# PrioteasaAndrei/music-style-transfer-ldm

Measured on AMD Instinct MI355X. Metric: UNet denoising steps/sec on 1×128×512 mel-latents, 1/2/4/8 MI355X, higher is better.
Workload: dtype fp32; 1 GPU; config 2: 50-step DDIM reverse sample (49 UNet+update iterations per step), batch 8/GPU, 1x128x512 mel -> [8,32,16,64] latents, eta=0.0, hipGraph replay of 1 concurrent sub-batch chains; global_batch=8, parallelism=dp1 (batch shards)

## Files before the change

include/ldm_capi.h:

```cpp
#ifndef LDM_CAPI_H
#define LDM_CAPI_H

#include <stddef.h>
#include <stdint.h>

#ifdef __cplusplus
extern "C" {
#endif

#define LDM_CAPI_VERSION 1

const char* ldm_last_error(void);
int ldm_capi_version(void);
int ldm_device_count(int* count);

typedef struct ldm_conv_desc {
    int32_t B, Cin, Hin, Win;
    int32_t Cout, Hout, Wout;
    int32_t kh, kw, stride, pad, out_pad;
    int32_t transposed;
    int32_t layout;
} ldm_conv_desc;

enum {
// ... 19 lines not shown
    float bn_eps;
    int32_t act;
    const float* bcast_add;
    const float* skip_add;
    float* act_out;
    int32_t dtype;
} ldm_epilogue;

typedef struct ldm_conv_plan {
    int32_t kind;
    int32_t tm, tn, wk;
    int32_t ks;
    int32_t balance;
    int64_t packed_floats;
    int64_t ws_floats;
} ldm_conv_plan;

int ldm_conv_make_plan(const ldm_conv_desc* d, ldm_conv_plan* plan);
int ldm_conv_tiled_plan(const ldm_conv_desc* d, int32_t dtype, ldm_conv_plan* plan);
int ldm_conv_sconv_plan(const ldm_conv_desc* d, int32_t dtype, ldm_conv_plan* plan);
int ldm_conv_make_plan_forced(const ldm_conv_desc* d, int kind, int tm, int tn, int wk, int ks,
                              ldm_conv_plan* plan);
int ldm_conv_pack_weight(const ldm_conv_desc* d, const ldm_conv_plan* plan, const float* w,
                         float* packed, void* stream);
int32_t ldm_conv_storage16(const ldm_conv_desc* d, const ldm_conv_plan* plan);
int ldm_conv_forward(const ldm_conv_desc* d, const ldm_conv_plan* plan, const float* x, const float* w,
                     const ldm_epilogue* ep, float* y, void* stream);
int ldm_conv_forward_ws(const ldm_conv_desc* d, const ldm_conv_plan* plan, const float* x, const float* w,
                        const ldm_epilogue* ep, float* y, float* workspace, void* stream);

int64_t ldm_reduce_workspace_floats(int32_t B, int32_t C, int32_t HW);
int ldm_batchnorm_train(float* x, int32_t B, int32_t C, int32_t HW, const float* weight, const float* bias,
                        float* running_mean, float* running_var, float momentum, float eps, int32_t act,
                        float* save_mean, float* save_invstd, float* workspace, void* stream);
int ldm_batchnorm_train_out(const float* x, float* y, int32_t B, int32_t C, int32_t HW, const float* weight,
                            const float* bias, float* running_mean, float* running_var, float momentum, float eps,
                            int32_t act, float* save_mean, float* save_invstd, float* workspace, void* stream);
int ldm_batchnorm_stats(const float* x, int32_t B, int32_t C, int32_t HW, double* stats, float* workspace,
                        void* stream);
int ldm_batchnorm_stats_code(const float* x, int32_t code, int32_t B, int32_t C, int32_t HW, double* stats,
                             float* workspace, void* stream);
int ldm_batchnorm_apply(float* x, int32_t B, int32_t C, int32_t HW, const double* stats, double count,
                        const float* weight, const float* bias, float* running_mean, float* running_var,
                        float momentum, float eps, int32_t act, float* save_mean, float* save_invstd, void* stream);
int ldm_batchnorm_apply_out(const float* x, float* y, int32_t B, int32_t C, int32_t HW, const double* stats,
                            double count, const float* weight, const float* bias, float* running_mean,
                            float* running_var, float momentum, float eps, int32_t act, float* save_mean,
                            float* save_invstd, void* stream);

int ldm_batchnorm_eval(const float* x, float* y, int32_t B, int32_t C, int32_t HW, const float* weight,
                       const float* bias, const float* running_mean, const float* running_var, float eps, int32_t act,
                       void* stream);

int ldm_activation(const float* x, float* y, int64_t n, int32_t act, void* stream);

int ldm_sinusoid_embed(const void* t, int32_t t_is_float, int32_t B, int32_t dim, const float* freqs, float* out,
                       void* stream);

int ldm_time_mlp_forward(const void* t, int32_t t_is_float, int32_t B, int32_t dim, const float* freqs,
                         const float* w1, const float* b1, const float* w2, const float* b2, float* out,
                         void* stream);

int ldm_attention_fold_keys(const float* kv, const float* wq, const float* bq, int32_t B, int32_t E, int32_t heads,
                            int32_t S, float scale, float* kf, float* bf, void* stream);
int ldm_attention_folded(const float* z, const float* kv, const float* kf, const float* bf, float* out, int32_t B,
                         int32_t E, int32_t heads, int32_t L, int32_t S, void* stream);
int ldm_attention_folded_keys(const float* z, const float* kv, const float* kf, const float* bf,
                              const float* key_bias, float* out, int32_t B, int32_t E, int32_t heads, int32_t L,
                              int32_t S, void* stream);
int ldm_attention_fold_keys_bias(const float* kv, const float* wq, const float* bq, int32_t B, int32_t E,
                                 int32_t heads, int32_t S, float scale, const float* key_bias, float* kf, float* bf,
                                 void* stream);
int ldm_attention_folded_probs(const float* z, const float* kf, const float* bf, float* p, int32_t B, int32_t E,
                               int32_t heads, int32_t L, int32_t S, void* stream);
int32_t ldm_bneck_fold_supported(int32_t B, int32_t H, int32_t W);
int ldm_bneck_fold_values(const float* w_fold, const float* kv, float* u, int32_t B, void* stream);
int ldm_bneck_pv(const float* u, const float* p, const float* pos_bias, float* y, int32_t B, int32_t dtype,
                 void* stream);
int ldm_ca1_probs(const float* z4, const float* kf, const float* bf, float* p, int32_t B, void* stream);
int32_t ldm_ca1_probs_form(void);
int ldm_set_cin1_packed(int on);
int ldm_set_cin1_s1(int on);
int ldm_set_flash_split(int on);
int ldm_fold_conv_proj(const ldm_conv_desc* d, const float* w_conv, const float* b_conv, const float* w_proj,
                       const float* b_proj, int32_t Cmid, float* w_out, float* pos_bias_out, void* stream);
int ldm_attention_core(const float* q, const float* kv, float* out, int32_t B, int32_t E, int32_t heads,
                       int32_t L, int32_t S, float scale, void* stream);
int ldm_attention_flash_supported(int32_t E, int32_t heads);
int ldm_attention_forward_lse(const float* q, const float* kv, float* out, float* lse, int32_t B, int32_t E,
                              int32_t heads, int32_t L, int32_t S, float scale, void* stream);

int ldm_q_sample(const float* x0, const float* eps, const float* coef_table, int32_t T, const int64_t* t, float* zt,
                 int32_t B, int64_t per_sample, void* stream);
int ldm_predict_start(const float* zt, const float* eps, const float* coef_table, int32_t T, const int64_t* t,
                      float* x0, int32_t B, int64_t per_sample, void* stream);
int ldm_sched_backward(int32_t kind, const float* grad, const float* coef_table, int32_t T, const int64_t* t,
                       float* grad_a, float* grad_b, int32_t B, int64_t per_sample, void* stream);
int ldm_ddim_step(float* x, const float* eps, const float* coef, float eta, float* x0_log, float* eps_log,
                  int64_t n, void* stream);
int ldm_msolver_step(float* x, const float* eps, const float* coef, const float* x0_prev, float* x0_log,
                     float* eps_log, int64_t n, void* stream);

int ldm_loss_forward(int32_t kind, const float* a, const float* b, int64_t n, void* workspace, float* out,
                     void* stream);
int ldm_loss_backward(int32_t kind, const float* a, const float* b, int64_t n, const float* grad_out, float* grad_a,
                      float* grad_b, void* stream);

typedef struct ldm_unet_weights {
    const float* conv_w[9];
    const float* conv_b[9];
    ldm_conv_plan conv_plan[9];
    const float* ca_wq[2];
    const float* ca_bq[2];
    ldm_conv_plan ca_plan_q[2];
    const float* ca_wkv[2];
    const float* ca_bkv[2];
    ldm_conv_plan ca_plan_kv[2];
    const float* ca_wo[2];
    const float* ca_bo[2];
    ldm_conv_plan ca_plan_o[2];
    const float* t_freqs;
    const float* t_w1;
    const float* t_b1;
    const float* t_w2;
    const float* t_b2;
    const float* ca_wq_raw[2];
    const float* fold_w[2];
    const float* fold_pb[2];
    int32_t use_fold;
    const float* step_w[9];
    const float* step_pb[2];
    int32_t use_step;
    int32_t step_dtype;
    const float* step_bneck_w;
} ldm_unet_weights;

typedef struct ldm_unet_shape {
    int32_t B, C, H, W;
    int32_t nf;
} ldm_unet_shape;

int64_t ldm_unet_workspace_floats(const ldm_unet_shape* s, const ldm_unet_weights* w);
int ldm_unet_make_plans(const ldm_unet_shape* s, ldm_unet_weights* w);
int ldm_unet_layer_desc(const ldm_unet_shape* s, int32_t layer, ldm_conv_desc* d);
int ldm_unet_forward(const ldm_unet_shape* s, const ldm_unet_weights* w, const float* z, const void* t,
                     int32_t t_is_float, const float* s5, const float* s6, float* out, float* workspace,
                     void* stream);

int64_t ldm_ddim_workspace_floats(const ldm_unet_shape* s, const ldm_unet_weights* w, int32_t nsteps);
int ldm_ddim_sample(const ldm_unet_shape* s, const ldm_unet_weights* w, float* x, const float* s5,
                    const float* s6, const int64_t* t_table, const float* coef_table, int32_t nsteps, float eta,
                    float* x0_logs, float* eps_logs, int64_t log_step_stride, float* workspace, void* stream);
int ldm_msolver_sample(const ldm_unet_shape* s, const ldm_unet_weights* w, float* x, const float* s5,
                       const float* s6, const int64_t* t_table, const float* coef_table, int32_t nsteps,
                       float* x0_logs, float* eps_logs, int64_t log_step_stride, float* workspace, void* stream);
int64_t ldm_ddim_workspace_floats_mix(const ldm_unet_shape* s, const ldm_unet_weights* w, int32_t nsteps, int32_t S5,
                                      int32_t S6);
int ldm_ddim_sample_mix(const ldm_unet_shape* s, const ldm_unet_weights* w, float* x, const float* s5,
                        const float* s6, int32_t S5, int32_t S6, const float* key_bias5, const float* key_bias6,
                        const int64_t* t_table, const float* coef_table, int32_t nsteps, float eta, float* x0_logs,
                        float* eps_logs, int64_t log_step_stride, float* workspace, void* stream);
int ldm_msolver_sample_mix(const ldm_unet_shape* s, const ldm_unet_weights* w, float* x, const float* s5,
                           const float* s6, int32_t S5, int32_t S6, const float* key_bias5, const float* key_bias6,
                           const int64_t* t_table, const float* coef_table, int32_t nsteps, float* x0_logs,
                           float* eps_logs, int64_t log_step_stride, float* workspace, void* stream);
int64_t ldm_ddim_workspace_floats_guided(const ldm_unet_shape* s, const ldm_unet_weights* w, int32_t nsteps, int32_t S5,
// ... 177 lines not shown
```

music-style-transfer-ldm_amd/csrc/misc.hip:

```cpp
#include <algorithm>

#include "common.h"

#pragma clang fp contract(off)

namespace ldm {

__global__ __launch_bounds__(256) void time_mlp_kernel(const void* t, int t_is_float, int dim, const float* __restrict__ freqs,
                                                       const float* __restrict__ w1, const float* __restrict__ b1,
                                                       const float* __restrict__ w2, const float* __restrict__ b2,
                                                       float* __restrict__ out) {
    extern __shared__ __attribute__((aligned(16))) float sm[];
    float* emb = sm;
    float* hid = sm + dim;
    const int b = blockIdx.x, i = threadIdx.x;
    const float tv = t_is_float ? ((const float*)t)[b] : (float)((const int64_t*)t)[b];
    const int half = dim / 2;
    if (i < dim) {
        const float arg = tv * freqs[i < half ? i : i - half];
        emb[i] = i < half ? sinf(arg) : cosf(arg);
    }
    __syncthreads();
    if (i < dim) {
        const float* wr = w1 + (size_t)i * dim;
// ... 232 lines not shown

#pragma unroll
        for (int r = 0; r < MF::NACC; ++r) Ps[(lt * TILE + MF::row(r, lg)) * LDP + st * TILE + col] = acc[r];
    }
    __syncthreads();
    {
        constexpr int RPW = SP >= 64 ? 1 : 64 / SP;
        constexpr int SEG = SP >= 64 ? 64 : SP;
        const int sub = lane / SEG, s0 = lane % SEG;
        for (int r0 = wave * RPW; r0 < LT; r0 += NW * RPW) {
            const int r = r0 + sub;
            float* row = Ps + r * LDP;
            float x[SP / SEG];
            float mx = -INFINITY;
#pragma unroll
            for (int u = 0; u < SP / SEG; ++u) {
                const int s = s0 + u * SEG;
                if constexpr (EQ > 0) {
                    float v = row[s];
#pragma unroll
                    for (int w = 1; w < NW; ++w) v = v + row[s + w * LT * LDP];
                    x[u] = v + (s < S ? bf[(size_t)(b * heads + h) * S + s] : 0.f);
                } else {
                    x[u] = row[s];
                }
                if (s < S) mx = fmaxf(mx, x[u]);
            }
#pragma unroll
            for (int o = SEG / 2; o > 0; o >>= 1) mx = fmaxf(mx, __shfl_xor(mx, o));
            float sum = 0.f;
#pragma unroll
            for (int u = 0; u < SP / SEG; ++u) {
                const int s = s0 + u * SEG;
                x[u] = s < S ? expf(x[u] - mx) : 0.f;
                sum += x[u];
            }
#pragma unroll
            for (int o = SEG / 2; o > 0; o >>= 1) sum += __shfl_xor(sum, o);
#pragma unroll
            for (int u = 0; u < SP / SEG; ++u) row[s0 + u * SEG] = l0 + r < L ? x[u] / sum : 0.f;
        }
    }
    __syncthreads();
    if constexpr (PONLY) {
        float* pb = out + ((size_t)(b * heads + h) * L + l0) * S;
        for (int e = threadIdx.x; e < LT * SP; e += 64 * NW) {
            const int r = e / SP, s = e % SP;
            if (l0 + r < L && s < S) pb[(size_t)r * S + s] = Ps[r * LDP + s];
        }
        return;
    }
    constexpr int NTC = D / TILE;
    float* ob = TOK ? out + (size_t)b * L * E + (size_t)h * D : out + ((size_t)b * E + (size_t)h * D) * L;
    for (int tile = wave; tile < NTC * NTL; tile += NW) {
        const int ct = tile / NTL, lt = tile % NTL;
        typename MF::acc_t acc;
#pragma unroll
        for (int r = 0; r < MF::NACC; ++r) acc[r] = 0.f;
        const float* va = Vs + (ct * TILE + col) * LDP + lg;
        const float* pb = Ps + (lt * TILE + col) * LDP + lg;
#pragma unroll
        for (int k0 = 0; k0 < SP; k0 += KBP * NLG) {
            float av[KBP], bv[KBP];
#pragma unroll
            for (int j = 0; j < KBP; ++j) {
                av[j] = va[k0 + NLG * j];
                bv[j] = pb[k0 + NLG * j];
            }
#pragma unroll
            for (int j = 0; j < KBP; ++j) acc = MF::mma(av[j], bv[j], acc);
        }
        const int l = l0 + lt * TILE + col;
        if (l < L) {
            if constexpr (TOK && KIND == 2) {
                *reinterpret_cast<float4*>(ob + (size_t)l * E + ct * TILE + 4 * lg) = make_float4(acc[0], acc[1], acc[2], acc[3]);
            } else {
#pragma unroll
                for (int r = 0; r < MF::NACC; ++r) ob[(ct * TILE + MF::row(r, lg)) * qcs + l * qls] = acc[r];
            }
        }
    }
}

__global__ __launch_bounds__(256) void attention_fold_keys_kernel(const float* __restrict__ kv, const float* __restrict__ wq,
                                                                  const float* __restrict__ bq, int B, int E, int heads,
                                                                  int S, float scale, float* __restrict__ kf,
                                                                  float* __restrict__ bf, int64_t first) {
    const int d = E / heads;
    const int64_t nk = (int64_t)B * heads * E * S;
    const int64_t idx = first + (int64_t)blockIdx.x * blockDim.x + threadIdx.x;
    if (idx < nk) {
        const int e = (int)(idx % E);
        int64_t r = idx / E;
        const int s = (int)(r % S);
        r /= S;
        const int h = (int)(r % heads), b = (int)(r / heads);
        const float* kr = kv + ((int64_t)b * 2 * E + (int64_t)h * d) * S + s;
        const float* wr = wq + (int64_t)h * d * E + e;
        double acc = 0.0;
        int c = 0;
        for (; c + 16 <= d; c += 16) {
            float wv[16], kvv[16];
#pragma unroll
            for (int u = 0; u < 16; ++u) {
                wv[u] = wr[(int64_t)(c + u) * E];
                kvv[u] = kr[(int64_t)(c + u) * S];
            }
#pragma unroll
            for (int u = 0; u < 16; ++u) acc += (double)wv[u] * (double)kvv[u];
        }
        for (; c < d; ++c) acc += (double)wr[(int64_t)c * E] * (double)kr[(int64_t)c * S];
        kf[idx] = (float)(acc * (double)scale);
    } else if (idx < nk + (int64_t)B * heads * S) {
        const int64_t j = idx - nk;
        const int s = (int)(j % S);
        const int bh = (int)(j / S);
        const int h = bh % heads, b = bh / heads;
        const float* kr = kv + ((int64_t)b * 2 * E + (int64_t)h * d) * S + s;
        double acc = 0.0;
        for (int c = 0; c < d; ++c) acc += (double)bq[h * d + c] * (double)kr[(int64_t)c * S];
        bf[j] = (float)(acc * (double)scale);
    }
}

__global__ __launch_bounds__(256) void attention_fold_keys4_kernel(const float* __restrict__ kv, const float* __restrict__ wq,
                                                                   const float* __restrict__ bq, int B, int E, int heads,
                                                                   int S, float scale, float* __restrict__ kf,
                                                                   float* __restrict__ bf) {
    const int d = E / heads;
    const int SG = S / 4;
    const int64_t n = (int64_t)B * heads * SG * (E + 1);
    const int64_t idx = (int64_t)blockIdx.x * blockDim.x + threadIdx.x;
    if (idx >= n) return;
    const int e = (int)(idx % (E + 1));
    int64_t r = idx / (E + 1);
    const int sg = (int)(r % SG);
    r /= SG;
    const int h = (int)(r % heads), b = (int)(r / heads);
    const float* kr = kv + ((int64_t)b * 2 * E + (int64_t)h * d) * S + sg * 4;
    const bool isb = e == E;
    const float* wr = isb ? bq + h * d : wq + (int64_t)h * d * E + e;
    const int64_t ws = isb ? 1 : E;
    double acc[4] = {0., 0., 0., 0.};
    int c = 0;
    for (; c + 16 <= d; c += 16) {
        float wv[16];
        float4 kq[16];
#pragma unroll
        for (int u = 0; u < 16; ++u) {
            wv[u] = wr[(int64_t)(c + u) * ws];
            kq[u] = *reinterpret_cast<const float4*>(kr + (int64_t)(c + u) * S);
        }
#pragma unroll
        for (int u = 0; u < 16; ++u) {
            const double w = (double)wv[u];
            acc[0] += w * (double)kq[u].x;
            acc[1] += w * (double)kq[u].y;
            acc[2] += w * (double)kq[u].z;
            acc[3] += w * (double)kq[u].w;
        }
    }
    for (; c < d; ++c) {
        const double w = (double)wr[(int64_t)c * ws];
        const float4 k = *reinterpret_cast<const float4*>(kr + (int64_t)c * S);
        acc[0] += w * (double)k.x;
        acc[1] += w * (double)k.y;
// ... 158 lines not shown
                                                       const float* __restrict__ freqs, float* __restrict__ out) {
    const int i = blockIdx.x * blockDim.x + threadIdx.x;
    if (i >= B * dim) return;
    const int b = i / dim, k = i - b * dim, half = dim / 2;
    const float tv = t_is_float ? ((const float*)t)[b] : (float)((const int64_t*)t)[b];
    const float arg = tv * freqs[k < half ? k : k - half];
    out[i] = k < half ? sinf(arg) : cosf(arg);
}

constexpr int kLossBlocks = 512;

__device__ __forceinline__ float loss_term(int kind, float a, float b) {
    if (kind == 0) {
        const float d = a - b;
        return d * d;
    }
    const float a2 = a * a;
    return 0.5f * ((a2 - 1.0f) - logf(a2 + 1e-8f));
}

__global__ __launch_bounds__(256) void loss_partial_kernel(int kind, const float* __restrict__ a,
                                                           const float* __restrict__ b, int64_t n,
                                                           double* __restrict__ partial) {
    __shared__ double red[16];
    double s = 0.0;
    for (int64_t i = (int64_t)blockIdx.x * blockDim.x + threadIdx.x; i < n; i += (int64_t)gridDim.x * blockDim.x)
        s += (double)loss_term(kind, a[i], b ? b[i] : 0.f);
    for (int o = 32; o > 0; o >>= 1) s += __shfl_xor(s, o);
    const int lane = threadIdx.x & 63, wave = threadIdx.x >> 6;
    if (lane == 0) red[wave] = s;
    __syncthreads();
    if (threadIdx.x == 0) {
        double t = 0.0;
        for (int w = 0; w < (int)(blockDim.x >> 6); ++w) t += red[w];
        partial[blockIdx.x] = t;
    }
}

__global__ __launch_bounds__(64) void loss_final_kernel(const double* __restrict__ partial, int np, int64_t n,
                                                        float* __restrict__ out) {
    double s = 0.0;
    for (int i = threadIdx.x; i < np; i += 64) s += partial[i];
    for (int o = 32; o > 0; o >>= 1) s += __shfl_xor(s, o);
    if (threadIdx.x == 0) out[0] = (float)(s / (double)n);
}

__global__ __launch_bounds__(256) void loss_backward_kernel(int kind, const float* __restrict__ a,
                                                            const float* __restrict__ b, int64_t n,
                                                            const float* __restrict__ g, float* __restrict__ ga,
                                                            float* __restrict__ gb) {
    const int64_t i = (int64_t)blockIdx.x * blockDim.x + threadIdx.x;
    if (i >= n) return;
    const float scale = g[0] / (float)n;
    if (kind == 0) {
        const float d = 2.0f * (a[i] - (b ? b[i] : 0.f)) * scale;
        if (ga) ga[i] = d;
        if (gb) gb[i] = -d;
    } else {
        const float av = a[i];
        const float a2 = av * av;
        if (ga) ga[i] = (av - av / (a2 + 1e-8f)) * scale;
    }
}

static unsigned blocks_for(int64_t n, int t) { return (unsigned)((n + t - 1) / t); }

}

using namespace ldm;

extern "C" int ldm_time_mlp_forward(const void* t, int32_t t_is_float, int32_t B, int32_t dim, const float* freqs,
                                    const float* w1, const float* b1, const float* w2, const float* b2, float* out,
                                    void* stream) {
    LDM_REQUIRE(t && freqs && w1 && b1 && w2 && b2 && out, "time_mlp: null argument");
    LDM_REQUIRE(B > 0 && dim > 1 && dim % 2 == 0 && dim <= 256, "time_mlp: unsupported dim");
    const int threads = (dim + 63) / 64 * 64;
    hipLaunchKernelGGL(time_mlp_kernel, dim3(B), dim3(threads), 2 * dim * sizeof(float), (hipStream_t)stream, t,
                       t_is_float, dim, freqs, w1, b1, w2, b2, out);
    LDM_CHECK_LAUNCH("time_mlp_kernel");
    return 0;
}

namespace ldm {
int attention_folded(const float* z, const float* kv, const float* kf, const float* bf, float* out, int32_t B,
                     int32_t E, int32_t heads, int32_t L, int32_t S, hipStream_t st) {
    LDM_REQUIRE(z && kv && kf && bf && out, "attention (folded): null argument");
    LDM_REQUIRE(B > 0 && heads == 4 && L > 0 && S > 0, "attention (folded): bad shape");
    const int d = E / heads;
#define LDM_ATTF(LP, SP, D, LT, EQV, NWV)                                                                \
    if (d == D && E == EQV && L <= LP && S <= SP) {                                                      \
        const size_t lds = ((size_t)NWV * LT * (SP + 1) + (size_t)D * (SP + 1)) * sizeof(float);       \
        if (lds > 64 * 1024) {                                                                           \
            static bool opted = false;                                                                   \
            if (!opted) {                                                                                \
                LDM_HIP_TRY(hipFuncSetAttribute(                                                         \
                    (const void*)attention_mfma_kernel<2, LP, SP, D, LT, true, EQV, NWV>,                  \
                    hipFuncAttributeMaxDynamicSharedMemorySize, 160 * 1024));                            \
                opted = true;                                                                            \
            }                                                                                            \
        }                                                                                                \
        hipLaunchKernelGGL((attention_mfma_kernel<2, LP, SP, D, LT, true, EQV, NWV>), dim3(B * heads * (LP / LT)), \
                           dim3(64 * NWV), lds, st, z, kv, out, E, heads, L, S, 1.0f, kf, bf);           \
        LDM_CHECK_LAUNCH("attention_mfma_kernel (folded)");                                              \
        return 0;                                                                                        \
    }
    LDM_ATTF(16, 16, 128, 16, 512, 8)
    LDM_ATTF(64, 64, 64, 16, 256, 16)
    LDM_ATTF(32, 32, 64, 16, 256, 8)
    LDM_ATTF(32, 32, 128, 16, 512, 8)
    LDM_ATTF(16, 16, 64, 16, 256, 4)
#undef LDM_ATTF
    return fail(3, "attention (folded): no instance for this shape");
}

int attention_folded_probs(const float* z, const float* kf, const float* bf, float* p, int32_t B, int32_t E,
                           int32_t heads, int32_t L, int32_t S, hipStream_t st) {
    LDM_REQUIRE(z && kf && bf && p, "attention probs (folded): null argument");
    LDM_REQUIRE(B > 0 && heads == 4 && E == 512 && L > 0 && L <= 16 && S > 0 && S <= 16,
                "attention probs (folded): instances for CA1's 2 x 8 plane only (E 512, L, S <= 16)");
    static const int nw = [] {
        const char* e = std::getenv("LDM_CA1P_WAVES");
        return e && std::atoi(e) == 16 ? 16 : 8;
    }();
    if (nw == 16) {
        auto kfn = attention_mfma_kernel<2, 16, 16, 128, 16, true, 512, 16, true>;
        const size_t lds = ((size_t)16 * 16 * 17 + (size_t)128 * 17) * sizeof(float);
        hipLaunchKernelGGL(kfn, dim3(B * heads), dim3(64 * 16), lds, st, z, kf, p, E, heads, L, S, 1.0f, kf, bf);
    } else {
        auto kfn = attention_mfma_kernel<2, 16, 16, 128, 16, true, 512, 8, true>;
        const size_t lds = ((size_t)8 * 16 * 17 + (size_t)128 * 17) * sizeof(float);
        hipLaunchKernelGGL(kfn, dim3(B * heads), dim3(64 * 8), lds, st, z, kf, p, E, heads, L, S, 1.0f, kf, bf);
    }
    LDM_CHECK_LAUNCH("attention_mfma_kernel (folded, probabilities)");
    return 0;
}

int attention_fold_keys(const float* kv, const float* wq, const float* bq, int32_t B, int32_t E, int32_t heads,
                        int32_t S, float scale, float* kf, float* bf, hipStream_t st) {
    LDM_REQUIRE(kv && wq && bq && kf && bf && B > 0 && heads > 0 && E % heads == 0 && S > 0, "fold keys: bad argument");
    const int64_t nk = (int64_t)B * heads * E * S, nb = (int64_t)B * heads * S;
    static const bool k4_on = [] {
        const char* e = std::getenv("LDM_FOLD_KEYS4");
        return e ? std::atoi(e) != 0 : true;
    }();
    const bool k4 = k4_on && S % 4 == 0 && ((uintptr_t)kv & 15) == 0;
    if (k4) {
        const int64_t n4 = (int64_t)B * heads * (S / 4) * (E + 1);
        hipLaunchKernelGGL(attention_fold_keys4_kernel, dim3((unsigned)((n4 + 255) / 256)), dim3(256), 0, st, kv, wq, bq,
                           B, E, heads, S, scale, kf, bf);
        LDM_CHECK_LAUNCH("attention_fold_keys4_kernel");
        return 0;
    }
    const int64_t first = 0, n = nk + nb - first;
    hipLaunchKernelGGL(attention_fold_keys_kernel, dim3((unsigned)((n + 255) / 256)), dim3(256), 0, st, kv, wq, bq, B,
                       E, heads, S, scale, kf, bf, first);
    LDM_CHECK_LAUNCH("attention_fold_keys_kernel");
    return 0;
}

int attention_core_ex(const float* q, const float* kv, float* out, int32_t B, int32_t E, int32_t heads, int32_t L,
                      int32_t S, float scale, bool tok, hipStream_t st) {
    LDM_REQUIRE(q && kv && out, "attention: null argument");
    LDM_REQUIRE(B > 0 && heads > 0 && E % heads == 0 && L > 0 && S > 0, "attention: bad shape");
    const int d = E / heads;
    {
        const dim3 blk(256);
#define LDM_ATT(KIND, LP, SP, D, LT)                                                                      \
    if (d == D && L <= LP && S <= SP) {                                                                   \
        const size_t lds = ((size_t)LT * (SP + 1) + (size_t)D * (SP + 1)) * sizeof(float);              \
        if (tok)                                                                                          \
            hipLaunchKernelGGL((attention_mfma_kernel<KIND, LP, SP, D, LT, true>), dim3(B * heads * (LP / LT)), blk, \
// ... 69 lines not shown
    return 0;
}

extern "C" int ldm_msolver_step(float* x, const float* eps, const float* coef, const float* x0_prev, float* x0_log,
                                float* eps_log, int64_t n, void* stream) {
    LDM_REQUIRE(x && eps && coef && x0_log && n > 0, "msolver_step: bad argument");
    LDM_REQUIRE(x0_prev != x0_log, "msolver_step: x0_prev must not be the x0 output");
    hipLaunchKernelGGL(msolver_step_kernel, dim3(blocks_for(n, 256)), dim3(256), 0, (hipStream_t)stream, x, eps, coef,
                       x0_prev, x0_log, eps_log, n);
    LDM_CHECK_LAUNCH("msolver_step_kernel");
    return 0;
}

extern "C" int ldm_guide_eps(const float* e_t, const float* e_b, const float* scale, int64_t per_sample, int32_t B,
                             float* out, void* stream) {
    LDM_REQUIRE(e_t && e_b && scale && out && per_sample > 0 && B > 0, "guide_eps: bad argument");
    const int64_t n = per_sample * B;
    hipLaunchKernelGGL(guide_eps_kernel, dim3(blocks_for(n, 256)), dim3(256), 0, (hipStream_t)stream, e_t, e_b, scale,
                       per_sample, n, out);
    LDM_CHECK_LAUNCH("guide_eps_kernel");
    return 0;
}

extern "C" int ldm_activation(const float* x, float* y, int64_t n, int32_t act, void* stream) {
    LDM_REQUIRE(x && y && n >= 0, "activation: bad argument");
    if (n == 0) return 0;
    hipLaunchKernelGGL(activation_kernel, dim3(blocks_for(n, 256)), dim3(256), 0, (hipStream_t)stream, x, y, n, act);
    LDM_CHECK_LAUNCH("activation_kernel");
    return 0;
}

extern "C" int ldm_batchnorm_eval(const float* x, float* y, int32_t B, int32_t C, int32_t HW, const float* weight,
                                  const float* bias, const float* running_mean, const float* running_var, float eps,
                                  int32_t act, void* stream) {
    LDM_REQUIRE(x && y && running_mean && running_var && B > 0 && C > 0 && HW > 0, "batchnorm_eval: bad argument");
    const int64_t n = (int64_t)B * C * HW;
    hipLaunchKernelGGL(batchnorm_eval_kernel, dim3(blocks_for(n, 256)), dim3(256), 0, (hipStream_t)stream, x, y, C, HW,
                       n, weight, bias, running_mean, running_var, eps, act);
    LDM_CHECK_LAUNCH("batchnorm_eval_kernel");
    return 0;
}

extern "C" int ldm_sinusoid_embed(const void* t, int32_t t_is_float, int32_t B, int32_t dim, const float* freqs,
                                  float* out, void* stream) {
    LDM_REQUIRE(t && freqs && out && B > 0 && dim > 1 && dim % 2 == 0, "sinusoid: bad argument");
    hipLaunchKernelGGL(sinusoid_kernel, dim3(blocks_for((int64_t)B * dim, 256)), dim3(256), 0, (hipStream_t)stream, t,
                       t_is_float, B, dim, freqs, out);
    LDM_CHECK_LAUNCH("sinusoid_kernel");
    return 0;
}

extern "C" int ldm_loss_forward(int32_t kind, const float* a, const float* b, int64_t n, void* workspace, float* out,
                                void* stream) {
    LDM_REQUIRE(a && workspace && out && n > 0 && (kind == 0 || kind == 1), "loss_forward: bad argument");
    LDM_REQUIRE(kind != 0 || b, "loss_forward: mse needs two inputs");
    const int np = (int)std::min<int64_t>(kLossBlocks, (n + 255) / 256);
    hipLaunchKernelGGL(loss_partial_kernel, dim3(np), dim3(256), 0, (hipStream_t)stream, kind, a, b, n,
                       (double*)workspace);
    LDM_CHECK_LAUNCH("loss_partial_kernel");
    hipLaunchKernelGGL(loss_final_kernel, dim3(1), dim3(64), 0, (hipStream_t)stream, (const double*)workspace, np, n, out);
    LDM_CHECK_LAUNCH("loss_final_kernel");
    return 0;
}

extern "C" int ldm_loss_backward(int32_t kind, const float* a, const float* b, int64_t n, const float* grad_out,
                                 float* grad_a, float* grad_b, void* stream) {
    LDM_REQUIRE(a && grad_out && n > 0 && (kind == 0 || kind == 1), "loss_backward: bad argument");
    hipLaunchKernelGGL(loss_backward_kernel, dim3(blocks_for(n, 256)), dim3(256), 0, (hipStream_t)stream, kind, a, b, n,
                       grad_out, grad_a, grad_b);
    LDM_CHECK_LAUNCH("loss_backward_kernel");
    return 0;
}

extern "C" int ldm_attention_fold_keys(const float* kv, const float* wq, const float* bq, int32_t B, int32_t E,
                                       int32_t heads, int32_t S, float scale, float* kf, float* bf, void* stream) {
    return ldm::attention_fold_keys(kv, wq, bq, B, E, heads, S, scale, kf, bf, (hipStream_t)stream);
}

extern "C" int ldm_attention_folded(const float* z, const float* kv, const float* kf, const float* bf, float* out,
                                    int32_t B, int32_t E, int32_t heads, int32_t L, int32_t S, void* stream) {
    return ldm::attention_folded(z, kv, kf, bf, out, B, E, heads, L, S, (hipStream_t)stream);
}

extern "C" int ldm_attention_folded_probs(const float* z, const float* kf, const float* bf, float* p, int32_t B,
                                          int32_t E, int32_t heads, int32_t L, int32_t S, void* stream) {
    return ldm::attention_folded_probs(z, kf, bf, p, B, E, heads, L, S, (hipStream_t)stream);
}

extern "C" int ldm_fold_conv_proj(const ldm_conv_desc* d, const float* w_conv, const float* b_conv, const float* w_proj,
                                  const float* b_proj, int32_t Cmid, float* w_out, float* pos_bias_out, void* stream) {
    LDM_REQUIRE(d && w_conv && w_proj && b_proj && w_out && pos_bias_out, "fold conv/proj: null argument");
    LDM_REQUIRE(!d->transposed && d->kh * d->kw > 0 && Cmid > 0, "fold conv/proj: a plain conv after the projection");
    const int64_t n = (int64_t)d->Cout * d->Cin * d->kh * d->kw + (int64_t)d->Cout * d->Hout * d->Wout;
    hipLaunchKernelGGL(ldm::fold_conv_proj_kernel, dim3((unsigned)((n + 255) / 256)), dim3(256), 0, (hipStream_t)stream,
                       w_conv, b_conv, w_proj, b_proj, d->Cout, Cmid, d->Cin, d->kh, d->kw, d->stride, d->pad, d->Hin,
                       d->Win, d->Hout, d->Wout, w_out, pos_bias_out);
    LDM_CHECK_LAUNCH("fold_conv_proj_kernel");
    return 0;
}
```

music-style-transfer-ldm_amd/ldm_amd/_lib.py:

```python
import ctypes
import os

import torch

PKG_ROOT = os.path.dirname(os.path.dirname(os.path.abspath(__file__)))
LIB_PATH = os.environ.get("LDM_AMD_LIB", os.path.join(PKG_ROOT, "lib", "libldm_amd.so"))

c_int32 = ctypes.c_int32
c_int64 = ctypes.c_int64
c_float = ctypes.c_float
c_vp = ctypes.c_void_p
c_fp = ctypes.c_void_p


class ConvDesc(ctypes.Structure):
    _fields_ = [(n, c_int32) for n in
                ("B", "Cin", "Hin", "Win", "Cout", "Hout", "Wout", "kh", "kw", "stride", "pad", "out_pad", "transposed",
                 "layout")]

    def key(self):
        return tuple(getattr(self, f[0]) for f in self._fields_)


class Epilogue(ctypes.Structure):
# ... 62 lines not shown
    "ldm_step_layer_forms": (c_int32, [c_vp]),
    "ldm_step_dec1_ddim": (c_int32, [c_int32, c_int32, c_int32, c_fp, c_fp, c_fp, c_fp, c_float, c_fp, c_fp, c_fp,
                                     c_int32, c_vp]),
    "ldm_step_dec1_msolver": (c_int32, [c_int32, c_int32, c_int32, c_fp, c_fp, c_fp, c_fp, c_fp, c_fp, c_fp, c_fp,
                                        c_int32, c_vp]),
    "ldm_step_conv_ws": (c_int32, [c_int32, c_int32, c_int32, c_int32, c_fp, c_fp, c_fp, c_fp, c_fp, c_fp, c_int32,
                                   c_fp, c_vp]),
    "ldm_mel_quantize": (c_int32, [c_fp, c_fp, c_int64, ctypes.c_float, c_vp]),
    "ldm_mel_dequantize": (c_int32, [c_fp, c_fp, c_int64, ctypes.c_float, c_vp]),
    "ldm_u8_to_unit": (c_int32, [c_fp, c_fp, c_int64, c_vp]),
    "ldm_stft_table_floats": (c_int64, [c_int32]),
    "ldm_stft_fill_tables": (c_int32, [c_int32, c_vp]),
    "ldm_stft": (c_int32, [c_fp, c_int32, c_int64, c_int32, c_int32, c_fp, c_fp, c_fp, c_int32, c_vp]),
    "ldm_istft": (c_int32, [c_fp, c_fp, c_fp, c_int32, c_int32, c_int64, c_int32, c_int32, c_fp, c_vp]),
    "ldm_griffinlim_workspace": (c_int64, [c_int32, c_int32, c_int32]),
    "ldm_griffinlim": (c_int32, [c_fp, c_fp, c_fp, c_int32, c_int32, c_int64, c_int32, c_int32, c_int32, c_float,
                                 c_fp, c_fp, c_vp]),
    "ldm_mel_project": (c_int32, [c_fp, c_fp, c_vp, c_fp, c_int32, c_int32, c_int32, c_int32, c_vp]),
    "ldm_power_to_db": (c_int32, [c_fp, c_fp, c_int32, c_int64, c_float, c_float, c_fp, c_vp]),
    "ldm_db_to_power": (c_int32, [c_fp, c_fp, c_int64, c_vp]),
    "ldm_mel_invert": (c_int32, [c_fp, c_fp, c_fp, c_fp, c_vp, c_float, c_int32, c_int32, c_fp, c_fp, c_int32,
                                 c_int32, c_int32, c_int32, c_vp]),
    "ldm_resample_out_len": (c_int64, [c_int64, c_int32, c_int32]),
    "ldm_resample_f32": (c_int32, [c_fp, c_int32, c_int64, c_fp, c_int32, c_int32, c_int32, c_fp, c_vp]),
    "ldm_resample_pcm16": (c_int32, [c_vp, c_int64, c_int32, c_fp, c_int32, c_int32, c_int32, c_fp, c_vp]),
    "ldm_trim_workspace_floats": (c_int64, [c_int32, c_int64, c_int32]),
    "ldm_trim_bounds": (c_int32, [c_fp, c_int32, c_int64, c_int32, c_int32, c_float, c_fp, c_vp, c_vp]),
    "ldm_mel_window_count": (c_int64, [c_int64, c_int32, c_int32]),
    "ldm_mel_windows": (c_int32, [c_fp, c_int32, c_int64, c_int32, c_int32, c_float, c_float, c_float, c_fp, c_fp,
                                  c_vp]),
    "ldm_mel_stitch": (c_int32, [c_fp, c_fp, c_int32, c_int32, c_int32, c_int32, c_int64, c_float, c_fp, c_fp, c_vp]),
    "ldm_batchnorm_train": (c_int32, [c_fp, c_int32, c_int32, c_int32, c_fp, c_fp, c_fp, c_fp, c_float, c_float,
                                      c_int32, c_fp, c_fp, c_fp, c_vp]),
    "ldm_batchnorm_train_out": (c_int32, [c_fp, c_fp, c_int32, c_int32, c_int32, c_fp, c_fp, c_fp, c_fp, c_float,
                                          c_float, c_int32, c_fp, c_fp, c_fp, c_vp]),
    "ldm_batchnorm_apply_out": (c_int32, [c_fp, c_fp, c_int32, c_int32, c_int32, c_vp, ctypes.c_double, c_fp, c_fp,
                                          c_fp, c_fp, c_float, c_float, c_int32, c_fp, c_fp, c_vp]),
    "ldm_maxpool2x2": (c_int32, [c_fp, c_fp, c_int32, c_int32, c_int32, c_int32, c_vp]),
    "ldm_std_mse_workspace_floats": (c_int64, [c_int32, c_int64]),
    "ldm_std_mse_moments": (c_int32, [c_fp, c_fp, c_int32, c_int64, c_vp, c_fp, c_vp]),
    "ldm_std_mse_accumulate": (c_int32, [c_vp, c_int32, c_int64, ctypes.c_double, ctypes.c_double, c_vp, c_fp, c_vp]),
    "ldm_batchnorm_stats": (c_int32, [c_fp, c_int32, c_int32, c_int32, c_vp, c_fp, c_vp]),
    "ldm_batchnorm_apply": (c_int32, [c_fp, c_int32, c_int32, c_int32, c_vp, ctypes.c_double, c_fp, c_fp, c_fp, c_fp,
                                      c_float, c_float, c_int32, c_fp, c_fp, c_vp]),
    "ldm_batchnorm_eval": (c_int32, [c_fp, c_fp, c_int32, c_int32, c_int32, c_fp, c_fp, c_fp, c_fp, c_float, c_int32,
                                     c_vp]),
    "ldm_activation": (c_int32, [c_fp, c_fp, c_int64, c_int32, c_vp]),
    "ldm_sinusoid_embed": (c_int32, [c_vp, c_int32, c_int32, c_int32, c_fp, c_fp, c_vp]),
    "ldm_time_mlp_forward": (c_int32, [c_vp, c_int32, c_int32, c_int32, c_fp, c_fp, c_fp, c_fp, c_fp, c_fp, c_vp]),
    "ldm_attention_core": (c_int32, [c_fp, c_fp, c_fp, c_int32, c_int32, c_int32, c_int32, c_int32, c_float, c_vp]),
    "ldm_attention_flash_supported": (c_int32, [c_int32, c_int32]),
    "ldm_attention_forward_lse": (c_int32, [c_fp, c_fp, c_fp, c_fp, c_int32, c_int32, c_int32, c_int32, c_int32,
                                            c_float, c_vp]),
    "ldm_attention_backward_flash": (c_int32, [c_fp, c_fp, c_fp, c_fp, c_fp, c_fp, c_fp, c_fp, c_int32, c_int32,
                                               c_int32, c_int32, c_int32, c_float, c_vp]),
    "ldm_pack_job_bytes": (c_int64, []),
    "ldm_pack_many_prepare": (c_int32, [ctypes.POINTER(ConvDesc), ctypes.POINTER(ConvPlan), ctypes.POINTER(c_vp),
                                        ctypes.POINTER(c_vp), c_int32, c_vp, ctypes.POINTER(c_int64)]),
    "ldm_pack_many": (c_int32, [c_vp, c_int32, c_int64, c_vp]),
    "ldm_im2col": (c_int32, [c_fp, c_int32, c_int32, c_int32, c_int32, c_int32, c_int32, c_int32, c_int32, c_int32,
                             c_fp, c_fp, c_int32, c_int32, c_fp, c_vp]),
    "ldm_col2im": (c_int32, [c_fp, c_int32, c_int32, c_int32, c_int32, c_int32, c_int32, c_int32, c_int32, c_int32,
                             c_fp, c_int32, c_int32, c_fp, c_vp]),
    "ldm_maxpool3s2": (c_int32, [c_fp, c_fp, c_int32, c_int32, c_int32, c_int32, c_vp]),
    "ldm_maxpool3s2_backward": (c_int32, [c_fp, c_fp, c_fp, c_int32, c_int32, c_int32, c_int32, c_vp]),
    "ldm_lpips_layer": (c_int32, [c_fp, c_fp, c_fp, c_int32, c_int32, c_int32, c_fp, c_fp, c_vp]),
    "ldm_lpips_layer_backward": (c_int32, [c_fp, c_fp, c_fp, c_fp, c_int32, c_int32, c_int32, c_int32, c_int32, c_fp,
                                           c_vp]),
    "ldm_attention_fold_keys": (c_int32, [c_fp, c_fp, c_fp, c_int32, c_int32, c_int32, c_int32, c_float, c_fp, c_fp,
                                          c_vp]),
    "ldm_attention_folded": (c_int32, [c_fp, c_fp, c_fp, c_fp, c_fp, c_int32, c_int32, c_int32, c_int32, c_int32,
                                       c_vp]),
    "ldm_fold_conv_proj": (c_int32, [ctypes.POINTER(ConvDesc), c_fp, c_fp, c_fp, c_fp, c_int32, c_fp, c_fp, c_vp]),
    "ldm_attention_folded_probs": (c_int32, [c_fp, c_fp, c_fp, c_fp, c_int32, c_int32, c_int32, c_int32, c_int32,
                                             c_vp]),
    "ldm_bneck_fold_supported": (c_int32, [c_int32, c_int32, c_int32]),
    "ldm_bneck_fold_values": (c_int32, [c_fp, c_fp, c_fp, c_int32, c_vp]),
    "ldm_bneck_pv": (c_int32, [c_fp, c_fp, c_fp, c_fp, c_int32, c_int32, c_vp]),
    "ldm_ca1_probs": (c_int32, [c_fp, c_fp, c_fp, c_fp, c_int32, c_vp]),
    "ldm_ca1_probs_form": (c_int32, []),
    "ldm_set_cin1_packed": (c_int32, [c_int32]),
    "ldm_set_cin1_s1": (c_int32, [c_int32]),
    "ldm_set_flash_split": (c_int32, [c_int32]),
    "ldm_q_sample": (c_int32, [c_fp, c_fp, c_fp, c_int32, c_vp, c_fp, c_int32, c_int64, c_vp]),
    "ldm_predict_start": (c_int32, [c_fp, c_fp, c_fp, c_int32, c_vp, c_fp, c_int32, c_int64, c_vp]),
    "ldm_sched_backward": (c_int32, [c_int32, c_fp, c_fp, c_int32, c_vp, c_fp, c_fp, c_int32, c_int64, c_vp]),
    "ldm_ddim_step":(c_int32, [c_fp, c_fp, c_fp, c_float, c_fp, c_fp, c_int64, c_vp]),
    "ldm_msolver_step": (c_int32, [c_fp, c_fp, c_fp, c_fp, c_fp, c_fp, c_int64, c_vp]),
    "ldm_loss_forward": (c_int32, [c_int32, c_fp, c_fp, c_int64, c_vp, c_fp, c_vp]),
    "ldm_loss_backward": (c_int32, [c_int32, c_fp, c_fp, c_int64, c_fp, c_fp, c_fp, c_vp]),
    "ldm_unet_workspace_floats": (c_int64, [ctypes.POINTER(UNetShape), ctypes.POINTER(UNetWeights)]),
    "ldm_ddim_workspace_floats": (c_int64, [ctypes.POINTER(UNetShape), ctypes.POINTER(UNetWeights), c_int32]),
    "ldm_unet_make_plans": (c_int32, [ctypes.POINTER(UNetShape), ctypes.POINTER(UNetWeights)]),
    "ldm_unet_layer_desc": (c_int32, [ctypes.POINTER(UNetShape), c_int32, ctypes.POINTER(ConvDesc)]),
    "ldm_unet_forward": (c_int32, [ctypes.POINTER(UNetShape), ctypes.POINTER(UNetWeights), c_fp, c_vp, c_int32,
                                   c_fp, c_fp, c_fp, c_fp, c_vp]),
    "ldm_ddim_sample": (c_int32, [ctypes.POINTER(UNetShape), ctypes.POINTER(UNetWeights), c_fp, c_fp, c_fp, c_vp,
                                  c_fp, c_int32, c_float, c_fp, c_fp, c_int64, c_fp, c_vp]),
    "ldm_msolver_sample": (c_int32, [ctypes.POINTER(UNetShape), ctypes.POINTER(UNetWeights), c_fp, c_fp, c_fp, c_vp,
                                     c_fp, c_int32, c_fp, c_fp, c_int64, c_fp, c_vp]),
    "ldm_attention_folded_keys": (c_int32, [c_fp, c_fp, c_fp, c_fp, c_fp, c_fp, c_int32, c_int32, c_int32, c_int32,
                                            c_int32, c_vp]),
    "ldm_attention_fold_keys_bias": (c_int32, [c_fp, c_fp, c_fp, c_int32, c_int32, c_int32, c_int32, c_float, c_fp,
                                               c_fp, c_fp, c_vp]),
    "ldm_ddim_workspace_floats_mix": (c_int64, [ctypes.POINTER(UNetShape), ctypes.POINTER(UNetWeights), c_int32,
                                                c_int32, c_int32]),
    "ldm_ddim_sample_mix": (c_int32, [ctypes.POINTER(UNetShape), ctypes.POINTER(UNetWeights), c_fp, c_fp, c_fp,
                                      c_int32, c_int32, c_fp, c_fp, c_vp, c_fp, c_int32, c_float, c_fp, c_fp, c_int64,
                                      c_fp, c_vp]),
    "ldm_msolver_sample_mix": (c_int32, [ctypes.POINTER(UNetShape), ctypes.POINTER(UNetWeights), c_fp, c_fp, c_fp,
                                         c_int32, c_int32, c_fp, c_fp, c_vp, c_fp, c_int32, c_fp, c_fp, c_int64, c_fp,
                                         c_vp]),
    "ldm_ddim_workspace_floats_guided": (c_int64, [ctypes.POINTER(UNetShape), ctypes.POINTER(UNetWeights), c_int32,
                                                   c_int32, c_int32]),
    "ldm_ddim_sample_guided": (c_int32, [ctypes.POINTER(UNetShape), ctypes.POINTER(UNetWeights), c_fp, c_fp, c_fp,
                                         c_fp, c_fp, c_int32, c_int32, c_fp, c_fp, c_fp, c_fp, c_fp, c_vp, c_fp,
                                         c_int32, c_float, c_fp, c_fp, c_int64, c_fp, c_vp]),
    "ldm_msolver_sample_guided": (c_int32, [ctypes.POINTER(UNetShape), ctypes.POINTER(UNetWeights), c_fp, c_fp, c_fp,
                                            c_fp, c_fp, c_int32, c_int32, c_fp, c_fp, c_fp, c_fp, c_fp, c_vp, c_fp,
                                            c_int32, c_fp, c_fp, c_int64, c_fp, c_vp]),
    "ldm_guide_eps": (c_int32, [c_fp, c_fp, c_fp, c_int64, c_int32, c_fp, c_vp]),
    "ldm_conv_tiled_plan": (c_int32, [ctypes.POINTER(ConvDesc), c_int32, ctypes.POINTER(ConvPlan)]),
    "ldm_conv_sconv_plan": (c_int32, [ctypes.POINTER(ConvDesc), c_int32, ctypes.POINTER(ConvPlan)]),
    "ldm_conv_storage16": (c_int32, [ctypes.POINTER(ConvDesc), ctypes.POINTER(ConvPlan)]),
    "ldm_conv_wgrad_storage16": (c_int32, [ctypes.POINTER(ConvDesc)]),
    "ldm_batchnorm_stats_code": (c_int32, [c_fp, c_int32, c_int32, c_int32, c_int32, c_vp, c_fp, c_vp]),
    "ldm_conv_wgrad_workspace_floats": (c_int64, [ctypes.POINTER(ConvDesc)]),
    "ldm_conv_backward_weight_dt": (c_int32, [ctypes.POINTER(ConvDesc), c_fp, c_fp, c_fp, c_int32, c_fp, c_int32, c_vp]),
    "ldm_conv_backward_weight": (c_int32, [ctypes.POINTER(ConvDesc), c_fp, c_fp, c_fp, c_int32, c_fp, c_vp]),
    "ldm_act_backward_defer": (c_int32, [c_fp, c_fp, c_fp, c_int32, c_int32, c_int32, c_int32, c_fp, c_fp, c_fp, c_vp,
                                         c_vp]),
    "ldm_act_partial_floats": (c_int64, [c_int32, c_int32, c_int32]),
    "ldm_batchnorm_backward_dxsum_defer": (c_int32, [c_fp, c_fp, c_fp, c_fp, c_fp, c_fp, c_fp, c_int32, c_int32, c_int32,
                                                     c_int32, c_fp, c_fp, c_fp, c_fp, c_vp, c_vp, c_fp, c_vp]),
    "ldm_bn_dxsum_partial_floats": (c_int64, [c_int32, c_int32, c_int32]),
    "ldm_conv_backward_weight_defer": (c_int32, [c_vp, c_fp, c_fp, c_fp, c_int32, c_fp, c_int32, c_vp, c_vp]),
    "ldm_wgrad_reduce_many": (c_int32, [c_vp, c_int32, c_vp]),
    "ldm_act_finalize_many": (c_int32, [c_vp, c_int32, c_vp]),
    "ldm_act_backward": (c_int32, [c_fp, c_fp, c_fp, c_int32, c_int32, c_int32, c_int32, c_fp, c_fp, c_fp, c_fp,
                                   c_vp]),
    "ldm_batchnorm_backward": (c_int32, [c_fp, c_fp, c_fp, c_fp, c_fp, c_fp, c_fp, c_int32, c_int32, c_int32,
                                         c_int32, c_fp, c_fp, c_fp, c_fp, c_vp]),
    "ldm_batchnorm_backward_dxsum": (c_int32, [c_fp, c_fp, c_fp, c_fp, c_fp, c_fp, c_fp, c_int32, c_int32, c_int32,
                                               c_int32, c_fp, c_fp, c_fp, c_fp, c_fp, c_vp]),
    "ldm_batchnorm_backward_reduce": (c_int32, [c_fp, c_fp, c_fp, c_fp, c_fp, c_fp, c_fp, c_int32, c_int32, c_int32,
                                                c_int32, c_vp, c_fp, c_fp, c_fp, c_vp]),
    "ldm_batchnorm_backward_apply": (c_int32, [c_fp, c_fp, c_fp, c_fp, c_fp, c_fp, c_fp, c_int32, c_int32, c_int32,
                                               c_int32, c_vp, ctypes.c_double, c_fp, c_vp]),
    "ldm_attention_backward": (c_int32, [c_fp, c_fp, c_fp, c_fp, c_fp, c_int32, c_int32, c_int32, c_int32, c_int32,
                                         c_float, c_vp]),
    "ldm_unscale_check": (c_int32, [c_vp, c_vp, c_vp, c_int32, c_int32, c_fp, c_vp, c_vp]),
    "ldm_adam_step": (c_int32, [c_vp, c_vp, c_vp, c_int32, c_int32, ctypes.c_double, ctypes.c_double,
                                ctypes.c_double, ctypes.c_double, ctypes.c_double, c_int32, c_int32, c_vp, c_vp]),
    "ldm_adam_step_dev": (c_int32, [c_vp, c_vp, c_vp, c_int32, c_int32, ctypes.c_double, ctypes.c_double,
                                    ctypes.c_double, ctypes.c_double, ctypes.c_double, c_int32, c_fp, c_vp, c_fp,
                                    c_vp]),
    "ldm_update_scale": (c_int32, [c_fp, c_vp, c_vp, c_float, c_float, c_int32, c_vp]),
}

TENSOR_SLOT_WORDS = 5

_LIB = None


class LDMError(RuntimeError):
    pass
# ... 37 lines not shown
```

Baseline: 14610 steps/s.

## Add specialized MFMA cross-attention kernel for E=256, L=S=64 folded attention

```diff
diff --git a/include/ldm_capi.h b/include/ldm_capi.h
--- a/include/ldm_capi.h
+++ b/include/ldm_capi.h
@@ -125,6 +125,8 @@
 int ldm_set_cin1_packed(int on);
 int ldm_set_cin1_s1(int on);
 int ldm_set_flash_split(int on);
+int ldm_set_ca2_form(int on);
+int32_t ldm_ca2_form(void);
 int ldm_fold_conv_proj(const ldm_conv_desc* d, const float* w_conv, const float* b_conv, const float* w_proj,
                        const float* b_proj, int32_t Cmid, float* w_out, float* pos_bias_out, void* stream);
 int ldm_attention_core(const float* q, const float* kv, float* out, int32_t B, int32_t E, int32_t heads,
diff --git a/music-style-transfer-ldm_amd/csrc/misc.hip b/music-style-transfer-ldm_amd/csrc/misc.hip
--- a/music-style-transfer-ldm_amd/csrc/misc.hip
+++ b/music-style-transfer-ldm_amd/csrc/misc.hip
@@ -338,6 +338,77 @@
     }
 }
 
+namespace ca2 {
+constexpr int E = 256, HEADS = 4, D = 64, L = 64, S = 64, LT = 16, NW = 16, LDP = 68;
+constexpr size_t kLds = ((size_t)NW * LT * S + (size_t)LT * LDP) * sizeof(float);
+}
+
+__global__ __launch_bounds__(64 * ca2::NW) void ca2_attn_kernel(const float* __restrict__ z, const float* __restrict__ kv,
+                                                                const float* __restrict__ kf,
+                                                                const float* __restrict__ bf, float* __restrict__ out) {
+    using namespace ca2;
+    extern __shared__ __attribute__((aligned(16))) float sm[];
+    float* slab = sm;
+    float* Ps = sm + NW * LT * S;
+    const int l0 = (blockIdx.x % (L / LT)) * LT;
+    const int bh = blockIdx.x / (L / LT);
+    const int h = bh % HEADS, b = bh / HEADS;
+    const int lane = threadIdx.x & 63;
+    const int wave = __builtin_amdgcn_readfirstlane(threadIdx.x >> 6);
+    const int col = lane & 15, lg = lane >> 4;
+    const int ct = wave >> 2, kq = wave & 3;
+    const int kbase = wave * (E / NW);
+    const floatx4 zz = *reinterpret_cast<const floatx4*>(z + ((size_t)b * L + l0 + col) * E + kbase + 4 * lg);
+    const float* kb = kf + (size_t)bh * S * E + (size_t)col * E + kbase + 4 * lg;
+    floatx4 kk[S / 16];
+#pragma unroll
+    for (int st = 0; st < S / 16; ++st) kk[st] = *reinterpret_cast<const floatx4*>(kb + (size_t)st * 16 * E);
+    const floatx4 vv = *reinterpret_cast<const floatx4*>(kv + ((size_t)b * 2 * E + E + (size_t)h * D + ct * 16 + col) * S +
+                                                          16 * kq + 4 * lg);
+    const float bias = bf[(size_t)bh * S + lane];
+    asm volatile("" ::"s"(out));
+    __builtin_amdgcn_sched_barrier(0);
+#pragma unroll
+    for (int st = 0; st < S / 16; ++st) {
+        floatx4 acc = {0.f, 0.f, 0.f, 0.f};
+#pragma unroll
+        for (int j = 0; j < 4; ++j) acc = __builtin_amdgcn_mfma_f32_16x16x4f32(zz[j], kk[st][j], acc, 0, 0, 0);
+#pragma unroll
+        for (int r = 0; r < 4; ++r) slab[(wave * LT + 4 * lg + r) * S + st * 16 + col] = acc[r];
+    }
+    __syncthreads();
+    {
+        float v = slab[wave * S + lane];
+#pragma unroll
+        for (int w = 1; w < NW; ++w) v = v + slab[(w * LT + wave) * S + lane];
+        const float x = v + bias;
+        float mx = fmaxf(-INFINITY, x);
+#pragma unroll
+        for (int o = 32; o > 0; o >>= 1) mx = fmaxf(mx, __shfl_xor(mx, o));
+        const float ex = expf(x - mx);
+        float sum = 0.f;
+        sum += ex;
+#pragma unroll
+        for (int o = 32; o > 0; o >>= 1) sum += __shfl_xor(sum, o);
+        Ps[wave * LDP + lane] = ex / sum;
+    }
+    __syncthreads();
+    {
+        const floatx4 pp = *reinterpret_cast<const floatx4*>(Ps + col * LDP + 16 * kq + 4 * lg);
+        floatx4 acc = {0.f, 0.f, 0.f, 0.f};
+#pragma unroll
+        for (int j = 0; j < 4; ++j) acc = __builtin_amdgcn_mfma_f32_16x16x4f32(vv[j], pp[j], acc, 0, 0, 0);
+        reinterpret_cast<floatx4*>(slab)[wave * 64 + lane] = acc;
+    }
+    __syncthreads();
+    if (kq != 0) return;
+    const floatx4* red = reinterpret_cast<const floatx4*>(slab) + wave * 64 + lane;
+    floatx4 o = red[0];
+#pragma unroll
+    for (int q = 1; q < 4; ++q) o = o + red[q * 64];
+    *reinterpret_cast<floatx4*>(out + ((size_t)b * L + l0 + col) * E + h * D + ct * 16 + 4 * lg) = o;
+}
+
 __global__ __launch_bounds__(256) void attention_fold_keys_kernel(const float* __restrict__ kv, const float* __restrict__ wq,
                                                                   const float* __restrict__ bq, int B, int E, int heads,
                                                                   int S, float scale, float* __restrict__ kf,
@@ -662,11 +733,30 @@
 }
 
 namespace ldm {
+static int g_ca2_form = [] {
+    const char* e = std::getenv("LDM_CA2_FORM");
+    return !e || std::atoi(e) != 0 ? 1 : 0;
+}();
+
 int attention_folded(const float* z, const float* kv, const float* kf, const float* bf, float* out, int32_t B,
                      int32_t E, int32_t heads, int32_t L, int32_t S, hipStream_t st) {
     LDM_REQUIRE(z && kv && kf && bf && out, "attention (folded): null argument");
     LDM_REQUIRE(B > 0 && heads == 4 && L > 0 && S > 0, "attention (folded): bad shape");
     const int d = E / heads;
+    if (g_ca2_form && E == ca2::E && L == ca2::L && S == ca2::S) {
+        LDM_REQUIRE((((uintptr_t)z | (uintptr_t)kv | (uintptr_t)kf | (uintptr_t)out) & 15) == 0,
+                    "attention (folded): operands must be 16-byte aligned");
+        static bool opted = false;
+        if (!opted) {
+            LDM_HIP_TRY(hipFuncSetAttribute((const void*)ca2_attn_kernel, hipFuncAttributeMaxDynamicSharedMemorySize,
+                                            160 * 1024));
+            opted = true;
+        }
+        hipLaunchKernelGGL(ca2_attn_kernel, dim3(B * ca2::HEADS * (ca2::L / ca2::LT)), dim3(64 * ca2::NW), ca2::kLds, st,
+                           z, kv, kf, bf, out);
+        LDM_CHECK_LAUNCH("ca2_attn_kernel");
+        return 0;
+    }
 #define LDM_ATTF(LP, SP, D, LT, EQV, NWV)                                                                \
     if (d == D && E == EQV && L <= LP && S <= SP) {                                                      \
         const size_t lds = ((size_t)NWV * LT * (SP + 1) + (size_t)D * (SP + 1)) * sizeof(float);       \
@@ -902,6 +992,14 @@
     return ldm::attention_folded(z, kv, kf, bf, out, B, E, heads, L, S, (hipStream_t)stream);
 }
 
+extern "C" int ldm_set_ca2_form(int on) {
+    const int prev = ldm::g_ca2_form;
+    ldm::g_ca2_form = on ? 1 : 0;
+    return prev;
+}
+
+extern "C" int32_t ldm_ca2_form(void) { return ldm::g_ca2_form; }
+
 extern "C" int ldm_attention_folded_probs(const float* z, const float* kf, const float* bf, float* p, int32_t B,
                                           int32_t E, int32_t heads, int32_t L, int32_t S, void* stream) {
     return ldm::attention_folded_probs(z, kf, bf, p, B, E, heads, L, S, (hipStream_t)stream);
diff --git a/music-style-transfer-ldm_amd/ldm_amd/_lib.py b/music-style-transfer-ldm_amd/ldm_amd/_lib.py
--- a/music-style-transfer-ldm_amd/ldm_amd/_lib.py
+++ b/music-style-transfer-ldm_amd/ldm_amd/_lib.py
@@ -168,6 +168,8 @@
     "ldm_set_cin1_packed": (c_int32, [c_int32]),
     "ldm_set_cin1_s1": (c_int32, [c_int32]),
     "ldm_set_flash_split": (c_int32, [c_int32]),
+    "ldm_set_ca2_form": (c_int32, [c_int32]),
+    "ldm_ca2_form": (c_int32, []),
     "ldm_q_sample": (c_int32, [c_fp, c_fp, c_fp, c_int32, c_vp, c_fp, c_int32, c_int64, c_vp]),
     "ldm_predict_start": (c_int32, [c_fp, c_fp, c_fp, c_int32, c_vp, c_fp, c_int32, c_int64, c_vp]),
     "ldm_sched_backward": (c_int32, [c_int32, c_fp, c_fp, c_int32, c_vp, c_fp, c_fp, c_int32, c_int64, c_vp]),
```

New measurement: 14750 steps/s, median of 6. No clear change (+1.0%).
